# faasm/faabric

Hardware: NVIDIA H100
Metric: mpi_allreduce_resnet50_grads_algbw_GBps (higher is better)
Workload: dtype int32

## Files before the change

### csrc/kernels/coll_group.cuh

```cuda
#pragma once

#include "fb_prims.cuh"
#include "launch_api.h"

namespace fb {

__device__ __forceinline__ bool groupEnter(const GroupArgs& a,
                                           GroupSeg* sSegs,
                                           BlockBarrier& bar)
{
    const Vec16* src = reinterpret_cast<const Vec16*>(a.segs);
    Vec16* dst = reinterpret_cast<Vec16*>(sSegs);
    for (uint32_t i = threadIdx.x; i < a.nSegs * 2; i += blockDim.x) {
        dst[i] = src[i];
    }
    bar.epoch = 0;
    if (!a.noSync) {
        bar.load(a.comm);
        return bar.sync(a.comm);
    }
    __syncthreads();
    return true;
}

__device__ __forceinline__ void groupExit(const GroupArgs& a, BlockBarrier& bar)
{
    if (!a.noSync) {
        bar.sync(a.comm);
        bar.store(a.comm);
    }
}

__device__ __forceinline__ int groupSegOf(const GroupSeg* s,
                                          uint32_t nSegs,
                                          int cur,
                                          uint32_t ch)
{
    if (s[cur].chunk0 <= ch && (cur + 1 == (int)nSegs || ch < s[cur + 1].chunk0)) {
        return cur;
    }
    int lo = 0;
    int hi = (int)nSegs - 1;
    while (lo < hi) {
        int mid = (lo + hi + 1) >> 1;
        if (s[mid].chunk0 <= ch) {
            lo = mid;
        } else {
            hi = mid - 1;
        }
    }
    return lo;
}

}
```

### csrc/kernels/coll_move.cu

```cuda
#include "coll_group.cuh"
#include "coll_move.cuh"

namespace fb {

template<int W>
struct Word;
template<>
struct Word<16>
{
    using type = Vec16;
    __device__ __forceinline__ static Vec16 ld(const uint8_t* p)
    {
        return ldVecStream(p);
    }
    __device__ __forceinline__ static void st(uint8_t* p, const Vec16& v)
    {
        stVec(p, v);
    }
};
template<>
struct Word<4>
{
    using type = uint32_t;
    __device__ __forceinline__ static uint32_t ld(const uint8_t* p)
// ... 157 lines not shown
                    const uint8_t* src = (p == a.root)
                                           ? a.comm.heap[p] + a.sendOff + b
                                           : a.comm.heap[p] + a.recvOff + b;
                    gridCopy<W>(a.comm.heap[rank] + a.recvOff + b,
                                src,
                                e - b,
                                tid,
                                nthreads);
                }
            }
        }
    }
    if (!a.noSync) {
        bar.sync(a.comm);
    }
    bar.store(a.comm);
}

template<int W>
static cudaError_t launchMoveW(const MoveArgs& a,
                               int blocks,
                               int threads,
                               cudaStream_t s)
{
    int n = a.comm.nranks;
    if (n == 2) {
        moveKernel<W, 2><<<blocks, threads, 0, s>>>(a);
    } else if (n == 4) {
        moveKernel<W, 4><<<blocks, threads, 0, s>>>(a);
    } else if (n == 8) {
        moveKernel<W, 8><<<blocks, threads, 0, s>>>(a);
    } else {
        moveKernel<W, 0><<<blocks, threads, 0, s>>>(a);
    }
    return cudaGetLastError();
}

cudaError_t launchMove(const MoveArgs& a,
                       int width,
                       int blocks,
                       int threads,
                       cudaStream_t s)
{
    if (width == 16) {
        return launchMoveW<16>(a, blocks, threads, s);
    }
    if (width == 4) {
        return launchMoveW<4>(a, blocks, threads, s);
    }
    return launchMoveW<1>(a, blocks, threads, s);
}

template<int NR>
__global__ void __launch_bounds__(512, 1) groupAllGatherKernel(const GroupArgs a)
{
    extern __shared__ __align__(16) uint8_t sGroupRaw[];
    GroupSeg* sSegs = reinterpret_cast<GroupSeg*>(sGroupRaw);
    const FbCommDev& c = a.comm;
    const int n = (NR > 0) ? NR : c.nranks;
    BlockBarrier bar;
    const bool ok = groupEnter(a, sSegs, bar);

    if (ok && a.nSegs > 0) {
        constexpr int UNROLL = (NR == 8) ? 2 : (NR == 1 ? 8 : 4);
        constexpr uint32_t CHUNK = 32u * UNROLL;
        const uint32_t lane = threadIdx.x & 31;
        const uint32_t warpsPerCta = blockDim.x >> 5;
        const uint32_t warpStride = gridDim.x * warpsPerCta;
        const uint8_t* const in = c.heap[c.rank];
        int cur = 0;
        for (uint32_t ch = blockIdx.x * warpsPerCta + (threadIdx.x >> 5);
             ch < a.totalChunks;
             ch += warpStride) {
            cur = groupSegOf(sSegs, a.nSegs, cur, ch);
            const GroupSeg sg = sSegs[cur];
            const uint32_t v0 = (ch - sg.chunk0) * CHUNK;
            const uint8_t* const src = in + sg.sendOff + (uint64_t)v0 * 16;
            const uint64_t rOff = sg.recvOff + (uint64_t)v0 * 16;
            const uint32_t rem = sg.nVec - v0;
            if (rem >= CHUNK) {
                Vec16 v[UNROLL];
#pragma unroll
                for (int u = 0; u < UNROLL; u++) {
                    v[u] = ldVecStream(src + (uint64_t)(u * 32 + lane) * 16);
                }
                if constexpr (NR > 0) {
#pragma unroll
                    for (int p = 0; p < NR; p++) {
#pragma unroll
                        for (int u = 0; u < UNROLL; u++) {
                            stVec(c.heap[p] + rOff + (uint64_t)(u * 32 + lane) * 16, v[u]);
                        }
                    }
                } else {
                    for (int p = 0; p < n; p++) {
#pragma unroll
                        for (int u = 0; u < UNROLL; u++) {
                            stVec(c.heap[p] + rOff + (uint64_t)(u * 32 + lane) * 16, v[u]);
                        }
                    }
                }
            } else {
#pragma unroll
                for (int u = 0; u < UNROLL; u++) {
                    const uint32_t i = (uint32_t)u * 32 + lane;
                    if (i < rem) {
                        const Vec16 v = ldVecStream(src + (uint64_t)i * 16);
                        for (int p = 0; p < n; p++) {
                            stVec(c.heap[p] + rOff + (uint64_t)i * 16, v);
                        }
                    }
                }
            }
        }
    }
    groupExit(a, bar);
}

cudaError_t launchGroupAllGather(const GroupArgs& a,
                                 int blocks,
                                 int threads,
                                 cudaStream_t s)
{
    const size_t smem = (size_t)a.nSegs * sizeof(GroupSeg);
    const int n = a.comm.nranks;
    if (n == 1) {
        groupAllGatherKernel<1><<<blocks, threads, smem, s>>>(a);
    } else if (n == 2) {
        groupAllGatherKernel<2><<<blocks, threads, smem, s>>>(a);
    } else if (n == 4) {
        groupAllGatherKernel<4><<<blocks, threads, smem, s>>>(a);
    } else if (n == 8) {
        groupAllGatherKernel<8><<<blocks, threads, smem, s>>>(a);
    } else {
        groupAllGatherKernel<0><<<blocks, threads, smem, s>>>(a);
    }
    return cudaGetLastError();
}

__global__ void barrierKernel(const FbCommDev c)
{
    BlockBarrier bar;
    bar.load(c);
    bar.sync(c);
    bar.store(c);
}

cudaError_t launchBarrier(const FbCommDev& c, cudaStream_t s)
{
    barrierKernel<<<1, 32, 0, s>>>(c);
    return cudaGetLastError();
}

__device__ __forceinline__ bool lastBlockDone(uint32_t* counter)
{
    __shared__ int sLast;
    __syncthreads();
    if (threadIdx.x == 0) {
        __threadfence();
        uint32_t prev = atomicAdd(counter, 1u);
        sLast = (prev == gridDim.x - 1) ? 1 : 0;
        if (sLast) {
            *counter = 0;
            __threadfence();
        }
    }
    __syncthreads();
    return sLast != 0;
}

template<int W>
__global__ void __launch_bounds__(512, 1) p2pSendKernel(const P2PArgs a)
{
    const FbCommDev& c = a.comm;
    const uint64_t tid = (uint64_t)blockIdx.x * blockDim.x + threadIdx.x;
    const uint64_t nthreads = (uint64_t)gridDim.x * blockDim.x;
    if (a.stage) {
        uint8_t* dst = c.heap[c.rank] + a.srcOff;
        const uint64_t lenW = a.bytes - (a.bytes % W);
        gridCopy<W>(dst, a.local, lenW, tid, nthreads);
        if (tid == 0) {
            for (uint64_t b = lenW; b < a.bytes; b++) {
                dst[b] = a.local[b];
            }
        }
    }
    uint32_t* done = c.sig[c.rank] + FB_P2P_DONE_OFF + a.peer;
    if (lastBlockDone(done) && threadIdx.x == 0) {
        uint32_t* desc = reinterpret_cast<uint32_t*>(c.heap[a.peer] + a.descOff) +
                         ((uint32_t)c.rank * FB_P2P_RING + (a.seq % FB_P2P_RING)) * 4;
// ... 188 lines not shown
```

### csrc/kernels/coll_reduce.cuh

```cuda
#pragma once

#include "coll_group.cuh"
#include "fb_prims.cuh"
#include "launch_api.h"

namespace fb {

template<typename VR, int NR>
__device__ __forceinline__ Vec16 gatherReduce(const ReduceArgs& a,
                                              uint64_t byteOff)
{
    if constexpr (NR > 0) {
        Vec16 v[NR];
#pragma unroll
        for (int p = 0; p < NR; p++) {
            v[p] = ldVecStream(a.comm.heap[p] + a.sendOff + byteOff);
        }
        Vec16 acc = v[0];
#pragma unroll
        for (int p = 1; p < NR; p++) {
            acc = VR::apply(acc, v[p]);
        }
        return acc;
    } else {
// ... 315 lines not shown
    } else {
        Vec16 v = ldVec(p);
        memcpy(&out, &v, 16);
    }
    return out;
}

template<typename E>
__device__ __forceinline__ void stElemGlobal(uint8_t* p, const E& in)
{
    if constexpr (sizeof(E) == 1) {
        uint8_t v;
        memcpy(&v, &in, 1);
        *reinterpret_cast<volatile uint8_t*>(p) = v;
    } else if constexpr (sizeof(E) == 2) {
        uint16_t v;
        memcpy(&v, &in, 2);
        *reinterpret_cast<volatile uint16_t*>(p) = v;
    } else if constexpr (sizeof(E) == 4) {
        uint32_t v;
        memcpy(&v, &in, 4);
        *reinterpret_cast<volatile uint32_t*>(p) = v;
    } else if constexpr (sizeof(E) == 8) {
        uint64_t v;
        memcpy(&v, &in, 8);
        *reinterpret_cast<volatile uint64_t*>(p) = v;
    } else {
        Vec16 v;
        memcpy(&v, &in, 16);
        stVec(p, v);
    }
}

template<typename VR>
__device__ __forceinline__ void groupTail(const FbCommDev& c,
                                          const GroupSeg& sg,
                                          int n)
{
    using Elem = typename VR::Elem;
    constexpr uint32_t EB = VR::ELEM_BYTES;
    const uint64_t base = (uint64_t)sg.nVec * 16;
    for (uint32_t e = 0; e + EB <= sg.tailBytes; e += EB) {
        Elem acc = ldElemGlobal<Elem>(c.heap[0] + sg.sendOff + base + e);
        for (int p = 1; p < n; p++) {
            Elem v = ldElemGlobal<Elem>(c.heap[p] + sg.sendOff + base + e);
            acc = VR::combine(acc, v);
        }
        for (int p = 0; p < n; p++) {
            stElemGlobal<Elem>(c.heap[p] + sg.recvOff + base + e, acc);
        }
    }
}

template<typename VR, int NR>
__global__ void __launch_bounds__(512, 1) groupAllReduceKernel(
  const GroupArgs a)
{
    extern __shared__ __align__(16) uint8_t sGroupRaw[];
    GroupSeg* sSegs = reinterpret_cast<GroupSeg*>(sGroupRaw);
    const FbCommDev& c = a.comm;
    const int n = (NR > 0) ? NR : c.nranks;
    {
        const Vec16* src = reinterpret_cast<const Vec16*>(a.segs);
        Vec16* dst = reinterpret_cast<Vec16*>(sGroupRaw);
        for (uint32_t i = threadIdx.x; i < a.nSegs * 2; i += blockDim.x) {
            dst[i] = src[i];
        }
    }
    BlockBarrier bar;
    bar.epoch = 0;
    bool ok = true;
    if (!a.noSync) {
        bar.load(c);
        ok = bar.sync(c);
    } else {
        __syncthreads();
    }

    if (ok && a.nSegs > 0) {
        constexpr int UNROLL = (NR == 8) ? 2 : (NR == 1 ? 8 : 4);
        constexpr uint32_t CHUNK = 32u * UNROLL;
        const uint32_t lane = threadIdx.x & 31;
        const uint32_t warpsPerCta = blockDim.x >> 5;
        const uint32_t warpStride = gridDim.x * warpsPerCta;
        int cur = 0;
        for (uint32_t ch = blockIdx.x * warpsPerCta + (threadIdx.x >> 5);
             ch < a.totalChunks;
             ch += warpStride) {
            if (!(sSegs[cur].chunk0 <= ch &&
                  (cur + 1 == (int)a.nSegs || ch < sSegs[cur + 1].chunk0))) {
                int lo = 0;
                int hi = (int)a.nSegs - 1;
                while (lo < hi) {
                    int mid = (lo + hi + 1) >> 1;
                    if (sSegs[mid].chunk0 <= ch) {
                        lo = mid;
                    } else {
                        hi = mid - 1;
                    }
                }
                cur = lo;
            }
            const GroupSeg sg = sSegs[cur];
            const uint32_t v0 = (ch - sg.chunk0) * CHUNK;
            const uint64_t sOff = sg.sendOff + (uint64_t)v0 * 16;
            const uint64_t rOff = sg.recvOff + (uint64_t)v0 * 16;
            const uint32_t rem = sg.nVec > v0 ? sg.nVec - v0 : 0;
            if (rem >= CHUNK) {
                Vec16 acc[UNROLL];
                if constexpr (NR > 0) {
                    Vec16 v[UNROLL][NR];
#pragma unroll
                    for (int u = 0; u < UNROLL; u++) {
#pragma unroll
                        for (int p = 0; p < NR; p++) {
                            v[u][p] = ldVecStream(c.heap[p] + sOff +
                                                  (uint64_t)(u * 32 + lane) * 16);
                        }
                    }
#pragma unroll
                    for (int u = 0; u < UNROLL; u++) {
                        acc[u] = v[u][0];
#pragma unroll
                        for (int p = 1; p < NR; p++) {
                            acc[u] = VR::apply(acc[u], v[u][p]);
                        }
                    }
#pragma unroll
                    for (int u = 0; u < UNROLL; u++) {
#pragma unroll
                        for (int p = 0; p < NR; p++) {
                            stVec(c.heap[p] + rOff + (uint64_t)(u * 32 + lane) * 16,
                                  acc[u]);
                        }
                    }
                } else {
#pragma unroll
                    for (int u = 0; u < UNROLL; u++) {
                        acc[u] = ldVecStream(c.heap[0] + sOff +
                                             (uint64_t)(u * 32 + lane) * 16);
                    }
                    for (int p = 1; p < n; p++) {
                        Vec16 v[UNROLL];
#pragma unroll
                        for (int u = 0; u < UNROLL; u++) {
                            v[u] = ldVecStream(c.heap[p] + sOff +
                                               (uint64_t)(u * 32 + lane) * 16);
                        }
#pragma unroll
                        for (int u = 0; u < UNROLL; u++) {
                            acc[u] = VR::apply(acc[u], v[u]);
                        }
                    }
                    for (int p = 0; p < n; p++) {
#pragma unroll
                        for (int u = 0; u < UNROLL; u++) {
                            stVec(c.heap[p] + rOff + (uint64_t)(u * 32 + lane) * 16,
                                  acc[u]);
                        }
                    }
                }
            } else {
#pragma unroll
                for (int u = 0; u < UNROLL; u++) {
                    const uint32_t i = (uint32_t)u * 32 + lane;
                    if (i < rem) {
                        Vec16 acc = ldVecStream(c.heap[0] + sOff + (uint64_t)i * 16);
                        for (int p = 1; p < n; p++) {
                            Vec16 v = ldVecStream(c.heap[p] + sOff + (uint64_t)i * 16);
                            acc = VR::apply(acc, v);
                        }
                        for (int p = 0; p < n; p++) {
                            stVec(c.heap[p] + rOff + (uint64_t)i * 16, acc);
                        }
                    }
                }
                if (sg.tailBytes != 0 && lane == 0 && v0 + CHUNK > sg.nVec) {
                    groupTail<VR>(c, sg, n);
                }
            }
        }
    }

    if (!a.noSync) {
        bar.sync(c);
        bar.store(c);
    }
}

template<typename VR>
cudaError_t launchGroup(const GroupArgs& a,
                        int blocks,
                        int threads,
                        cudaStream_t stream)
{
    const size_t smem = (size_t)a.nSegs * sizeof(GroupSeg);
    const int nr = a.comm.nranks;
    if (nr == 1) {
        groupAllReduceKernel<VR, 1><<<blocks, threads, smem, stream>>>(a);
    } else if (nr == 2) {
        groupAllReduceKernel<VR, 2><<<blocks, threads, smem, stream>>>(a);
    } else if (nr == 4) {
        groupAllReduceKernel<VR, 4><<<blocks, threads, smem, stream>>>(a);
    } else if (nr == 8) {
        groupAllReduceKernel<VR, 8><<<blocks, threads, smem, stream>>>(a);
    } else {
        groupAllReduceKernel<VR, 0><<<blocks, threads, smem, stream>>>(a);
    }
    return cudaGetLastError();
}

template<typename VR, int NR>
__global__ void __launch_bounds__(512, 1) groupReduceScatterKernel(
  const GroupArgs a)
{
    extern __shared__ __align__(16) uint8_t sGroupRaw[];
    GroupSeg* sSegs = reinterpret_cast<GroupSeg*>(sGroupRaw);
    const FbCommDev& c = a.comm;
    const int n = (NR > 0) ? NR : c.nranks;
    BlockBarrier bar;
    const bool ok = groupEnter(a, sSegs, bar);

    if (ok && a.nSegs > 0) {
        constexpr int UNROLL = (NR == 8) ? 2 : (NR == 1 ? 8 : 4);
        constexpr uint32_t CHUNK = 32u * UNROLL;
        const uint32_t lane = threadIdx.x & 31;
        const uint32_t warpsPerCta = blockDim.x >> 5;
        const uint32_t warpStride = gridDim.x * warpsPerCta;
        uint8_t* const out = c.heap[c.rank];
        int cur = 0;
        for (uint32_t ch = blockIdx.x * warpsPerCta + (threadIdx.x >> 5);
             ch < a.totalChunks;
             ch += warpStride) {
            cur = groupSegOf(sSegs, a.nSegs, cur, ch);
            const GroupSeg sg = sSegs[cur];
            const uint32_t v0 = (ch - sg.chunk0) * CHUNK;
            const uint64_t sOff = sg.sendOff + (uint64_t)v0 * 16;
            uint8_t* const dst = out + sg.recvOff + (uint64_t)v0 * 16;
            const uint32_t rem = sg.nVec - v0;
            if (rem >= CHUNK) {
                Vec16 acc[UNROLL];
                if constexpr (NR > 0) {
                    Vec16 v[UNROLL][NR];
#pragma unroll
                    for (int u = 0; u < UNROLL; u++) {
#pragma unroll
                        for (int p = 0; p < NR; p++) {
                            v[u][p] = ldVecStream(c.heap[p] + sOff +
                                                  (uint64_t)(u * 32 + lane) * 16);
                        }
                    }
#pragma unroll
                    for (int u = 0; u < UNROLL; u++) {
                        acc[u] = v[u][0];
#pragma unroll
                        for (int p = 1; p < NR; p++) {
                            acc[u] = VR::apply(acc[u], v[u][p]);
                        }
                    }
                } else {
#pragma unroll
                    for (int u = 0; u < UNROLL; u++) {
                        acc[u] = ldVecStream(c.heap[0] + sOff +
                                             (uint64_t)(u * 32 + lane) * 16);
                    }
                    for (int p = 1; p < n; p++) {
                        Vec16 v[UNROLL];
#pragma unroll
                        for (int u = 0; u < UNROLL; u++) {
                            v[u] = ldVecStream(c.heap[p] + sOff +
                                               (uint64_t)(u * 32 + lane) * 16);
                        }
#pragma unroll
                        for (int u = 0; u < UNROLL; u++) {
                            acc[u] = VR::apply(acc[u], v[u]);
                        }
                    }
                }
#pragma unroll
                for (int u = 0; u < UNROLL; u++) {
                    stVec(dst + (uint64_t)(u * 32 + lane) * 16, acc[u]);
                }
            } else {
#pragma unroll
                for (int u = 0; u < UNROLL; u++) {
                    const uint32_t i = (uint32_t)u * 32 + lane;
                    if (i < rem) {
                        Vec16 acc = ldVecStream(c.heap[0] + sOff + (uint64_t)i * 16);
                        for (int p = 1; p < n; p++) {
                            Vec16 v = ldVecStream(c.heap[p] + sOff + (uint64_t)i * 16);
                            acc = VR::apply(acc, v);
                        }
                        stVec(dst + (uint64_t)i * 16, acc);
                    }
                }
            }
        }
    }
    groupExit(a, bar);
}

template<typename VR>
cudaError_t launchGroupReduceScatter(const GroupArgs& a,
                                     int blocks,
                                     int threads,
                                     cudaStream_t stream)
{
    const size_t smem = (size_t)a.nSegs * sizeof(GroupSeg);
    const int nr = a.comm.nranks;
    if (nr == 1) {
        groupReduceScatterKernel<VR, 1><<<blocks, threads, smem, stream>>>(a);
    } else if (nr == 2) {
        groupReduceScatterKernel<VR, 2><<<blocks, threads, smem, stream>>>(a);
    } else if (nr == 4) {
        groupReduceScatterKernel<VR, 4><<<blocks, threads, smem, stream>>>(a);
    } else if (nr == 8) {
        groupReduceScatterKernel<VR, 8><<<blocks, threads, smem, stream>>>(a);
    } else {
        groupReduceScatterKernel<VR, 0><<<blocks, threads, smem, stream>>>(a);
    }
    return cudaGetLastError();
}

template<typename VR>
cudaError_t preloadReduce()
{
    cudaFuncAttributes a;
    cudaError_t e = cudaSuccess;
#define FB_PRELOAD(k)                                                          \
    if (e == cudaSuccess) {                                                    \
        e = cudaFuncGetAttributes(&a, k);                                      \
    }
    FB_PRELOAD((reduceKernel<VR, 0>))
    FB_PRELOAD((reduceKernel<VR, 2>))
    FB_PRELOAD((reduceKernel<VR, 4>))
    FB_PRELOAD((reduceKernel<VR, 8>))
    FB_PRELOAD((llAllReduceKernel<VR, 0>))
    FB_PRELOAD((llAllReduceKernel<VR, 2>))
    FB_PRELOAD((llAllReduceKernel<VR, 4>))
    FB_PRELOAD((llAllReduceKernel<VR, 8>))
    FB_PRELOAD((groupAllReduceKernel<VR, 0>))
    FB_PRELOAD((groupAllReduceKernel<VR, 1>))
    FB_PRELOAD((groupAllReduceKernel<VR, 2>))
    FB_PRELOAD((groupAllReduceKernel<VR, 4>))
    FB_PRELOAD((groupAllReduceKernel<VR, 8>))
    FB_PRELOAD((groupReduceScatterKernel<VR, 0>))
    FB_PRELOAD((groupReduceScatterKernel<VR, 1>))
    FB_PRELOAD((groupReduceScatterKernel<VR, 2>))
    FB_PRELOAD((groupReduceScatterKernel<VR, 4>))
    FB_PRELOAD((groupReduceScatterKernel<VR, 8>))
#undef FB_PRELOAD
    return e;
}

template<typename VR>
const ReduceLaunchers* launchersFor()
{
    static const ReduceLaunchers l = { &launchReduce<VR>,
                                       &launchLL<VR>,
                                       &launchGroup<VR>,
                                       &launchGroupReduceScatter<VR>,
                                       &preloadReduce<VR> };
    return &l;
}

}
```

### csrc/kernels/fb_prims.cuh

```cuda
#pragma once

#include <cuda_bf16.h>
#include <cuda_fp16.h>
#include <stdint.h>

#include <type_traits>

#include "faabric/device/comm_abi.h"

namespace fb {

__device__ __forceinline__ void stReleaseSys(uint32_t* p, uint32_t v)
{
    asm volatile("st.release.sys.global.u32 [%0], %1;" ::"l"(p), "r"(v)
                 : "memory");
}

__device__ __forceinline__ void stRelaxedSys(uint32_t* p, uint32_t v)
{
    asm volatile("st.relaxed.sys.global.u32 [%0], %1;" ::"l"(p), "r"(v)
                 : "memory");
}

__device__ __forceinline__ uint32_t ldAcquireSys(const uint32_t* p)
// ... 74 lines not shown

    __device__ __forceinline__ bool sync(const FbCommDev& c)
    {
        epoch += 1;
        __syncthreads();
        bool ok = true;
        if (threadIdx.x < (unsigned)c.nranks) {
            int peer = threadIdx.x;
            const size_t slot = (size_t)(c.blockBase + blockIdx.x);
            uint32_t* remote = c.sig[peer] + slot * FB_MAX_RANKS + c.rank;
            stReleaseSys(remote, epoch);
            const uint32_t* mine =
              c.sig[c.rank] + slot * FB_MAX_RANKS + peer;
            ok = waitFlagGe(c, mine, epoch, FB_ERR_BARRIER_TIMEOUT);
        }
        return __syncthreads_and(ok ? 1 : 0) != 0;
    }
};

struct alignas(16) Vec16
{
    uint32_t w[4];
};

__device__ __forceinline__ Vec16 ldVec(const void* p)
{
    Vec16 v;
    asm volatile("ld.global.v4.u32 {%0,%1,%2,%3}, [%4];"
                 : "=r"(v.w[0]), "=r"(v.w[1]), "=r"(v.w[2]), "=r"(v.w[3])
                 : "l"(p)
                 : "memory");
    return v;
}

__device__ __forceinline__ Vec16 ldVecStream(const void* p)
{
    Vec16 v;
    asm volatile(
      "ld.global.L1::no_allocate.v4.u32 {%0,%1,%2,%3}, [%4];"
      : "=r"(v.w[0]), "=r"(v.w[1]), "=r"(v.w[2]), "=r"(v.w[3])
      : "l"(p)
      : "memory");
    return v;
}

__device__ __forceinline__ void stVec(void* p, const Vec16& v)
{
    asm volatile("st.global.v4.u32 [%0], {%1,%2,%3,%4};" ::"l"(p),
                 "r"(v.w[0]),
                 "r"(v.w[1]),
                 "r"(v.w[2]),
                 "r"(v.w[3])
                 : "memory");
}

template<int OP>
struct OpTag
{
    static constexpr int value = OP;
};

template<typename T>
struct PairVI
{
    T v;
    int32_t i;
};

template<typename T, int OP>
struct Reducer
{
    __device__ __forceinline__ static T apply(T a, T b)
    {
        if constexpr (OP == FB_OP_MAX && std::is_same_v<T, float>) {
            return fmaxf(a, b);
        } else if constexpr (OP == FB_OP_MAX && std::is_same_v<T, double>) {
            return fmax(a, b);
        } else if constexpr (OP == FB_OP_MIN && std::is_same_v<T, float>) {
            return fminf(a, b);
        } else if constexpr (OP == FB_OP_MIN && std::is_same_v<T, double>) {
            return fmin(a, b);
        } else if constexpr (OP == FB_OP_MAX) {
            return a > b ? a : b;
        } else if constexpr (OP == FB_OP_MIN) {
            return a < b ? a : b;
        } else if constexpr (OP == FB_OP_SUM) {
            return a + b;
        } else if constexpr (OP == FB_OP_PROD) {
            return a * b;
        } else if constexpr (OP == FB_OP_LAND) {
            return (T)((a != (T)0) && (b != (T)0));
        } else if constexpr (OP == FB_OP_LOR) {
            return (T)((a != (T)0) || (b != (T)0));
        } else if constexpr (OP == FB_OP_LXOR) {
            return (T)((a != (T)0) != (b != (T)0));
        } else {
            return a;
        }
    }
};

template<typename T, int OP>
__device__ __forceinline__ T bitOp(T a, T b)
{
    if constexpr (OP == FB_OP_BAND) {
        return a & b;
// ... 29 lines not shown
{
    static constexpr bool value = true;
};

template<int OP>
struct IsBitwiseOp
{
    static constexpr bool value =
      (OP == FB_OP_BAND || OP == FB_OP_BOR || OP == FB_OP_BXOR);
};

template<typename H, int OP>
__device__ __forceinline__ H halfLikeApply(H a, H b)
{
    float r = Reducer<float, OP>::apply((float)a, (float)b);
    return (H)r;
}

template<typename T, int OP>
__device__ __forceinline__ T reduceElem(T a, T b)
{
    if constexpr (IsBitwiseOp<OP>::value) {
        if constexpr (IsFloatLike<T>::value) {
            return a;
        } else {
            return bitOp<T, OP>(a, b);
        }
    } else if constexpr (sizeof(T) == 2 && IsFloatLike<T>::value) {
        return halfLikeApply<T, OP>(a, b);
    } else {
        return Reducer<T, OP>::apply(a, b);
    }
}

template<typename T, int OP>
__device__ __forceinline__ PairVI<T> reducePair(PairVI<T> a, PairVI<T> b)
{
    if constexpr (OP == FB_OP_MAXLOC) {
        if (b.v > a.v || (b.v == a.v && b.i < a.i)) {
            return b;
        }
        return a;
    } else {
        if (b.v < a.v || (b.v == a.v && b.i < a.i)) {
            return b;
        }
        return a;
    }
}

template<typename T, int OP>
__device__ __forceinline__ Vec16 reduceVec(const Vec16& a, const Vec16& b)
{
    constexpr int N = 16 / sizeof(T);
    union U
    {
        Vec16 v;
        T e[N];
        __device__ U() {}
    };
    U ua, ub, ur;
    ua.v = a;
    ub.v = b;
#pragma unroll
    for (int i = 0; i < N; i++) {
        ur.e[i] = reduceElem<T, OP>(ua.e[i], ub.e[i]);
    }
    return ur.v;
}

template<typename T, int OP>
__device__ __forceinline__ Vec16 reduceVecPair(const Vec16& a, const Vec16& b)
{
    using P = PairVI<T>;
    constexpr int N = 16 / sizeof(P);
    union U
    {
        Vec16 v;
        P e[N];
        __device__ U() {}
    };
    U ua, ub, ur;
    ua.v = a;
    ub.v = b;
#pragma unroll
    for (int i = 0; i < N; i++) {
        ur.e[i] = reducePair<T, OP>(ua.e[i], ub.e[i]);
    }
    return ur.v;
}

template<typename T, bool PAIR>
struct ElemOf
{
    using type = T;
};
template<typename T>
struct ElemOf<T, true>
{
    using type = PairVI<T>;
};

template<typename T, int OP, bool PAIR>
struct VecReduce
{
    static constexpr int ELEM_BYTES = PAIR ? sizeof(PairVI<T>) : sizeof(T);
// ... 42 lines not shown
```

### csrc/kernels/launch_api.h

```cpp
#pragma once

#include <cuda_runtime.h>
#include <stdint.h>

#include "faabric/device/comm_abi.h"

namespace fb {

#define FB_NUM_SMS 132

struct ReduceArgs
{
    FbCommDev comm;
    uint64_t sendOff;
    uint64_t recvOff;
    uint8_t* recvLocal;
    uint64_t bytes;
    uint64_t vecBegin;
    uint64_t vecEnd;
    uint64_t outBase;
    int32_t readRanks;
    uint32_t pushMask;
    int32_t tailOwner;
    int32_t noSync;
};

typedef cudaError_t (*ReduceLaunchFn)(const ReduceArgs& a,
                                      int nr,
                                      int blocks,
                                      int threads,
                                      cudaStream_t stream);

#define FB_LL_BLOCKS 8
#define FB_LL_THREADS 512
#define FB_LL_MAX_VECS (FB_LL_BLOCKS * FB_LL_THREADS)
#define FB_LL_MAX_BYTES (FB_LL_MAX_VECS * 16)
#define FB_LL_AREA_BYTES(nranks) ((uint64_t)2 * (nranks) * FB_LL_MAX_VECS * 32)

struct LLArgs
{
    FbCommDev comm;
    const uint8_t* sendLocal;
    uint8_t* recvLocal;
    uint64_t bytes;
    uint64_t llOff;
    int32_t byteAccess;
    int32_t pad;
};

typedef cudaError_t (*LLLaunchFn)(const LLArgs& a, cudaStream_t stream);

struct GroupSeg
{
    uint64_t sendOff;
    uint64_t recvOff;
    uint32_t nVec;
    uint32_t chunk0;
    uint32_t tailBytes;
    uint32_t pad;
};

struct GroupArgs
{
    FbCommDev comm;
    const GroupSeg* segs;
    uint32_t nSegs;
    uint32_t totalChunks;
    int32_t noSync;
    int32_t pad;
};

static inline int fbGroupUnroll(int nranks)
{
    return (nranks == 8) ? 2 : (nranks == 1 ? 8 : 4);
}
static inline uint32_t fbGroupChunkVecs(int nranks)
{
    return 32u * (uint32_t)fbGroupUnroll(nranks);
}
#define FB_GROUP_MAX_SEGS 1024

typedef cudaError_t (*GroupLaunchFn)(const GroupArgs& a,
                                     int blocks,
                                     int threads,
                                     cudaStream_t stream);

cudaError_t launchGroupAllGather(const GroupArgs& a,
                                 int blocks,
                                 int threads,
                                 cudaStream_t stream);

struct ReduceLaunchers
{
    ReduceLaunchFn reduce;
    LLLaunchFn ll;
    GroupLaunchFn group;
    GroupLaunchFn groupRs;
    cudaError_t (*preload)();
};

const ReduceLaunchers* findReduceLaunchers(int dtype, int op);
const ReduceLaunchers* findReduceLaunchersInt(int dtype, int op);
const ReduceLaunchers* findReduceLaunchersFloat(int dtype, int op);
const ReduceLaunchers* findReduceLaunchersPair(int dtype, int op);


enum MoveMode
{
    MOVE_ALLGATHER = 0,
    MOVE_ALLTOALL = 1,
    MOVE_GATHER = 2,
    MOVE_SCATTER = 3,
    MOVE_BCAST = 4,
    MOVE_BCAST_2STEP = 5
};

struct MoveArgs
{
    FbCommDev comm;
    uint64_t sendOff;
    uint64_t recvOff;
    uint8_t* recvLocal;
    uint64_t chunkBytes;
    uint64_t srcStride;
    uint64_t dstStride;
    int32_t mode;
    int32_t root;
// ... 234 lines not shown
```

### csrc/src/device/communicator.cpp

```cpp
#include "faabric/device/communicator.h"
#include "faabric/device/nvtx.h"

#include "faabric/device/bootstrap.h"
#include "faabric/device/cuda_driver.h"
#include "launch_api.h"
#include "loopback_kernels.h"

#include <algorithm>
#include <chrono>
#include <thread>
#include <cstdio>
#include <initializer_list>
#include <barrier>
#include <cstdlib>
#include <cstring>
#include <set>
#include <shared_mutex>
#include <stdexcept>
#include <unistd.h>

namespace faabric::device {

#define CUDA_OK(expr)                                                          \
    do {                                                                       \
// ... 1892 lines not shown
        rc = FB_E_UNSUPPORTED;
        return nullptr;
    }
    const size_t esize = fbDtypeSize(dtype);
    if (esize == 0 || kind < GROUP_ALLREDUCE || kind > GROUP_ALLGATHER) {
        rc = FB_E_INVALID;
        return nullptr;
    }
    bindDevice();
    auto plan = std::make_shared<GroupPlan>();
    plan->kind = kind;
    plan->dtype = dtype;
    plan->device = device_;
    plan->items = nItems;
    for (size_t begin = 0; begin < nItems; begin += GROUP_ITEMS_PER_LAUNCH) {
        const size_t cnt = std::min(GROUP_ITEMS_PER_LAUNCH, nItems - begin);
        SegBuild sb;
        rc = buildSegs(*this, kind, items + begin, cnt, esize, sb);
        if (rc != FB_OK) {
            return nullptr;
        }
        GroupLaunch l;
        l.nSegs = (uint32_t)sb.segs.size();
        l.totalChunks = sb.totalChunks;
        l.vecsPerRank = sb.vecsPerRank;
        l.bytes = sb.bytes;
        const size_t tb = std::max<size_t>(sb.segs.size(), 1) * sizeof(fb::GroupSeg);
        if (loop_) {
            plan->hostTables = true;
            l.dSegs = (fb::GroupSeg*)::malloc(tb);
            if (!sb.segs.empty()) {
                memcpy(l.dSegs, sb.segs.data(), sb.segs.size() * sizeof(fb::GroupSeg));
            }
            plan->launches.push_back(l);
            continue;
        }
        if (cudaMalloc((void**)&l.dSegs, tb) != cudaSuccess) {
            cudaGetLastError();
            rc = FB_E_CUDA;
            return nullptr;
        }
        plan->launches.push_back(l);
        if (!sb.segs.empty() &&
            cudaMemcpy(l.dSegs, sb.segs.data(), sb.segs.size() * sizeof(fb::GroupSeg), cudaMemcpyHostToDevice) !=
              cudaSuccess) {
            cudaGetLastError();
            rc = FB_E_CUDA;
            return nullptr;
        }
    }
    return plan;
}

static int groupGrid(const CommConfig& cfg, int nranks, uint64_t vecsPerRank)
{
    const int slots = nranks == 1 ? 2 * FB_NUM_SMS : FB_MAX_BLOCKS / cfg.channels;
    const int cap = std::min(slots, cfg.groupBlocks > 0 ? cfg.groupBlocks : (nranks == 1 ? 2 * FB_NUM_SMS : 128));
    const uint64_t warps = (uint64_t)cfg.threads / 32;
    const uint64_t chunks = (vecsPerRank + fb::fbGroupChunkVecs(nranks) - 1) / fb::fbGroupChunkVecs(nranks);
    const uint64_t want = (chunks + warps * 2 - 1) / (warps * 2);
    return (int)std::clamp<uint64_t>(want, 1, (uint64_t)cap);
}

int Communicator::launchGroup(const GroupLaunch& l, GroupKind kind, int dtype, int op, int flags, cudaStream_t s)
{
    const int n = dev_.nranks;
    const bool ss = streamSync_ && !(flags & FB_FLAG_NOSYNC) && n > 1;
    fb::GroupArgs a;
    memset(&a, 0, sizeof(a));
    a.comm = devFor(flags);
    a.segs = l.dSegs;
    a.nSegs = l.nSegs;
    a.totalChunks = l.totalChunks;
    a.noSync = ((flags & FB_FLAG_NOSYNC) || ss || n == 1) ? 1 : 0;
    if (ss && streamBarrier(flags, s) != FB_OK) {
        return FB_E_CUDA;
    }
    const int blocks = groupGrid(cfg_, n, l.vecsPerRank);
    cudaError_t e;
    if (kind == GROUP_REDUCE_SCATTER) {
        e = k_->groupReduceScatter(a, dtype, op, blocks, cfg_.threads, s);
    } else if (kind == GROUP_ALLGATHER) {
        e = k_->groupAllGather(a, blocks, cfg_.threads, s);
    } else {
        e = k_->group(a, dtype, op, blocks, cfg_.threads, s);
    }
    if (e != cudaSuccess) {
        return FB_E_CUDA;
    }
    if (ss && streamBarrier(flags, s) != FB_OK) {
        return FB_E_CUDA;
    }
    stats_.launches++;
    stats_.bytes += l.bytes;
    if (kind == GROUP_ALLREDUCE) {
        stats_.algoCount[FB_ALGO_TWOSHOT]++;
    }
    return FB_OK;
}

int Communicator::allReduceGroup(const GroupPlan& plan, int op, int flags, cudaStream_t s)
{
    NvtxRange nvtxRange("fb::allReduceGroup");
    if (parent_ != nullptr) {
        return FB_E_UNSUPPORTED;
    }
    if (plan.kind != GROUP_ALLREDUCE) {
        return FB_E_INVALID;
    }
    const fb::ReduceLaunchers* L = fb::findReduceLaunchers(plan.dtype, op);
    if (L == nullptr || L->group == nullptr) {
        return FB_E_UNSUPPORTED;
    }
    bindDevice();
    for (const auto& l : plan.launches) {
        int rc = launchGroup(l, GROUP_ALLREDUCE, plan.dtype, op, flags, s);
        if (rc != FB_OK) {
            return rc;
        }
    }
    lastAlgo_ = FB_ALGO_TWOSHOT;
    return FB_OK;
}

int Communicator::reduceScatterGroup(const GroupPlan& plan, int op, int flags, cudaStream_t s)
{
    NvtxRange nvtxRange("fb::reduceScatterGroup");
    if (parent_ != nullptr) {
        return FB_E_UNSUPPORTED;
    }
    if (plan.kind != GROUP_REDUCE_SCATTER) {
// ... 938 lines not shown
```

Measured before the change: 1342.

## Unify group kernels with software-pipelined walk, PDL launch, and larger grids

Measured after the change: 1384, median of 6. 3.2% higher.

```diff
diff --git a/csrc/kernels/coll_group.cuh b/csrc/kernels/coll_group.cuh
--- a/csrc/kernels/coll_group.cuh
+++ b/csrc/kernels/coll_group.cuh
@@ -9,6 +9,8 @@
                                            GroupSeg* sSegs,
                                            BlockBarrier& bar)
 {
+    asm volatile("griddepcontrol.launch_dependents;" ::: "memory");
+    asm volatile("griddepcontrol.wait;" ::: "memory");
     const Vec16* src = reinterpret_cast<const Vec16*>(a.segs);
     Vec16* dst = reinterpret_cast<Vec16*>(sSegs);
     for (uint32_t i = threadIdx.x; i < a.nSegs * 2; i += blockDim.x) {
@@ -52,4 +54,85 @@
     return lo;
 }
 
+template<typename Kernel>
+cudaError_t launchGroupKernel(Kernel kernel,
+                              const GroupArgs& a,
+                              int blocks,
+                              int threads,
+                              size_t smem,
+                              cudaStream_t stream)
+{
+    cudaLaunchConfig_t cfg = {};
+    cfg.gridDim = dim3((unsigned)blocks);
+    cfg.blockDim = dim3((unsigned)threads);
+    cfg.dynamicSmemBytes = smem;
+    cfg.stream = stream;
+    cudaLaunchAttribute attr[1];
+    attr[0].id = cudaLaunchAttributeProgrammaticStreamSerialization;
+    attr[0].val.programmaticStreamSerializationAllowed = 1;
+    cfg.attrs = attr;
+    cfg.numAttrs = 1;
+    return cudaLaunchKernelEx(&cfg, kernel, a);
 }
+
+__host__ __device__ constexpr bool groupPipelined(int nr)
+{
+    return nr == 1 || nr == 2;
+}
+
+template<int U, int NR>
+struct GroupStage
+{
+    Vec16 v[U][NR > 0 ? NR : 1];
+};
+
+template<int U, bool PIPE, typename Stage, typename Load, typename Store, typename Ragged>
+__device__ __forceinline__ void groupWalk(const GroupArgs& a,
+                                          const GroupSeg* sSegs,
+                                          Load load,
+                                          Store store,
+                                          Ragged ragged)
+{
+    constexpr uint32_t CHUNK = 32u * U;
+    const uint32_t warpsPerCta = blockDim.x >> 5;
+    const uint32_t warpStride = gridDim.x * warpsPerCta;
+    Stage held;
+    uint64_t heldOff = 0;
+    bool have = false;
+    int cur = 0;
+    for (uint32_t ch = blockIdx.x * warpsPerCta + (threadIdx.x >> 5);
+         ch < a.totalChunks;
+         ch += warpStride) {
+        cur = groupSegOf(sSegs, a.nSegs, cur, ch);
+        const GroupSeg sg = sSegs[cur];
+        const uint32_t v0 = (ch - sg.chunk0) * CHUNK;
+        const uint32_t rem = sg.nVec > v0 ? sg.nVec - v0 : 0;
+        if (rem < CHUNK) {
+            ragged(sg, v0, rem);
+            continue;
+        }
+        const uint64_t sOff = sg.sendOff + (uint64_t)v0 * 16;
+        const uint64_t rOff = sg.recvOff + (uint64_t)v0 * 16;
+        if constexpr (PIPE) {
+            Stage next;
+            load(next, sOff);
+            if (have) {
+                store(held, heldOff);
+            }
+            held = next;
+            heldOff = rOff;
+            have = true;
+        } else {
+            Stage s;
+            load(s, sOff);
+            store(s, rOff);
+        }
+    }
+    if constexpr (PIPE) {
+        if (have) {
+            store(held, heldOff);
+        }
+    }
+}
+
+}
diff --git a/csrc/kernels/coll_move.cu b/csrc/kernels/coll_move.cu
--- a/csrc/kernels/coll_move.cu
+++ b/csrc/kernels/coll_move.cu
@@ -233,7 +233,8 @@
 }
 
 template<int NR>
-__global__ void __launch_bounds__(512, 1) groupAllGatherKernel(const GroupArgs a)
+__global__ void __launch_bounds__(512, groupPipelined(NR) ? 2 : 1) groupAllGatherKernel(
+  const GroupArgs a)
 {
     extern __shared__ __align__(16) uint8_t sGroupRaw[];
     GroupSeg* sSegs = reinterpret_cast<GroupSeg*>(sGroupRaw);
@@ -243,57 +244,40 @@
     const bool ok = groupEnter(a, sSegs, bar);
 
     if (ok && a.nSegs > 0) {
-        constexpr int UNROLL = (NR == 8) ? 2 : (NR == 1 ? 8 : 4);
-        constexpr uint32_t CHUNK = 32u * UNROLL;
+        constexpr int U = fbGroupUnroll(NR);
+        using Stage = GroupStage<U, 1>;
         const uint32_t lane = threadIdx.x & 31;
-        const uint32_t warpsPerCta = blockDim.x >> 5;
-        const uint32_t warpStride = gridDim.x * warpsPerCta;
         const uint8_t* const in = c.heap[c.rank];
-        int cur = 0;
-        for (uint32_t ch = blockIdx.x * warpsPerCta + (threadIdx.x >> 5);
-             ch < a.totalChunks;
-             ch += warpStride) {
-            cur = groupSegOf(sSegs, a.nSegs, cur, ch);
-            const GroupSeg sg = sSegs[cur];
-            const uint32_t v0 = (ch - sg.chunk0) * CHUNK;
-            const uint8_t* const src = in + sg.sendOff + (uint64_t)v0 * 16;
-            const uint64_t rOff = sg.recvOff + (uint64_t)v0 * 16;
-            const uint32_t rem = sg.nVec - v0;
-            if (rem >= CHUNK) {
-                Vec16 v[UNROLL];
-#pragma unroll
-                for (int u = 0; u < UNROLL; u++) {
-                    v[u] = ldVecStream(src + (uint64_t)(u * 32 + lane) * 16);
-                }
-                if constexpr (NR > 0) {
-#pragma unroll
-                    for (int p = 0; p < NR; p++) {
-#pragma unroll
-                        for (int u = 0; u < UNROLL; u++) {
-                            stVec(c.heap[p] + rOff + (uint64_t)(u * 32 + lane) * 16, v[u]);
-                        }
-                    }
-                } else {
-                    for (int p = 0; p < n; p++) {
-#pragma unroll
-                        for (int u = 0; u < UNROLL; u++) {
-                            stVec(c.heap[p] + rOff + (uint64_t)(u * 32 + lane) * 16, v[u]);
-                        }
-                    }
-                }
-            } else {
-#pragma unroll
-                for (int u = 0; u < UNROLL; u++) {
-                    const uint32_t i = (uint32_t)u * 32 + lane;
-                    if (i < rem) {
-                        const Vec16 v = ldVecStream(src + (uint64_t)i * 16);
-                        for (int p = 0; p < n; p++) {
-                            stVec(c.heap[p] + rOff + (uint64_t)i * 16, v);
-                        }
-                    }
-                }
-            }
-        }
+        groupWalk<U, groupPipelined(NR), Stage>(
+          a,
+          sSegs,
+          [&](Stage& s, uint64_t sOff) {
+#pragma unroll
+              for (int u = 0; u < U; u++) {
+                  s.v[u][0] = ldVecData(in + sOff + (uint64_t)(u * 32 + lane) * 16);
+              }
+          },
+          [&](const Stage& s, uint64_t rOff) {
+              for (int p = 0; p < n; p++) {
+#pragma unroll
+                  for (int u = 0; u < U; u++) {
+                      stVecData(c.heap[p] + rOff + (uint64_t)(u * 32 + lane) * 16, s.v[u][0]);
+                  }
+              }
+          },
+          [&](const GroupSeg& sg, uint32_t v0, uint32_t rem) {
+#pragma unroll
+              for (int u = 0; u < U; u++) {
+                  const uint32_t i = (uint32_t)u * 32 + lane;
+                  if (i < rem) {
+                      const uint64_t vOff = (uint64_t)(v0 + i) * 16;
+                      const Vec16 v = ldVecData(in + sg.sendOff + vOff);
+                      for (int p = 0; p < n; p++) {
+                          stVecData(c.heap[p] + sg.recvOff + vOff, v);
+                      }
+                  }
+              }
+          });
     }
     groupExit(a, bar);
 }
@@ -306,17 +290,16 @@
     const size_t smem = (size_t)a.nSegs * sizeof(GroupSeg);
     const int n = a.comm.nranks;
     if (n == 1) {
-        groupAllGatherKernel<1><<<blocks, threads, smem, s>>>(a);
+        return launchGroupKernel(groupAllGatherKernel<1>, a, blocks, threads, smem, s);
     } else if (n == 2) {
-        groupAllGatherKernel<2><<<blocks, threads, smem, s>>>(a);
+        return launchGroupKernel(groupAllGatherKernel<2>, a, blocks, threads, smem, s);
     } else if (n == 4) {
-        groupAllGatherKernel<4><<<blocks, threads, smem, s>>>(a);
+        return launchGroupKernel(groupAllGatherKernel<4>, a, blocks, threads, smem, s);
     } else if (n == 8) {
-        groupAllGatherKernel<8><<<blocks, threads, smem, s>>>(a);
+        return launchGroupKernel(groupAllGatherKernel<8>, a, blocks, threads, smem, s);
     } else {
-        groupAllGatherKernel<0><<<blocks, threads, smem, s>>>(a);
-    }
-    return cudaGetLastError();
+        return launchGroupKernel(groupAllGatherKernel<0>, a, blocks, threads, smem, s);
+    }
 }
 
 __global__ void barrierKernel(const FbCommDev c)
diff --git a/csrc/kernels/coll_reduce.cuh b/csrc/kernels/coll_reduce.cuh
--- a/csrc/kernels/coll_reduce.cuh
+++ b/csrc/kernels/coll_reduce.cuh
@@ -391,166 +391,63 @@
     }
 }
 
+template<typename VR, int NR, int U>
+__device__ __forceinline__ void groupGather(GroupStage<U, NR>& s,
+                                            const FbCommDev& c,
+                                            int n,
+                                            uint64_t off)
+{
+    const uint32_t lane = threadIdx.x & 31;
+    if constexpr (NR > 0) {
+#pragma unroll
+        for (int u = 0; u < U; u++) {
+#pragma unroll
+            for (int p = 0; p < NR; p++) {
+                s.v[u][p] = ldVecData(c.heap[p] + off + (uint64_t)(u * 32 + lane) * 16);
+            }
+        }
+    } else {
+#pragma unroll
+        for (int u = 0; u < U; u++) {
+            s.v[u][0] = ldVecData(c.heap[0] + off + (uint64_t)(u * 32 + lane) * 16);
+        }
+        for (int p = 1; p < n; p++) {
+            Vec16 v[U];
+#pragma unroll
+            for (int u = 0; u < U; u++) {
+                v[u] = ldVecData(c.heap[p] + off + (uint64_t)(u * 32 + lane) * 16);
+            }
+#pragma unroll
+            for (int u = 0; u < U; u++) {
+                s.v[u][0] = VR::apply(s.v[u][0], v[u]);
+            }
+        }
+    }
+}
+
+template<typename VR, int NR, int U>
+__device__ __forceinline__ Vec16 groupReduced(const GroupStage<U, NR>& s, int u)
+{
+    Vec16 acc = s.v[u][0];
+#pragma unroll
+    for (int p = 1; p < NR; p++) {
+        acc = VR::apply(acc, s.v[u][p]);
+    }
+    return acc;
+}
+
+template<typename VR>
+__device__ __forceinline__ Vec16 groupGatherOne(const FbCommDev& c, int n, uint64_t off)
+{
+    Vec16 acc = ldVecData(c.heap[0] + off);
+    for (int p = 1; p < n; p++) {
+        acc = VR::apply(acc, ldVecData(c.heap[p] + off));
+    }
+    return acc;
+}
+
 template<typename VR, int NR>
-__global__ void __launch_bounds__(512, 1) groupAllReduceKernel(
-  const GroupArgs a)
-{
-    extern __shared__ __align__(16) uint8_t sGroupRaw[];
-    GroupSeg* sSegs = reinterpret_cast<GroupSeg*>(sGroupRaw);
-    const FbCommDev& c = a.comm;
-    const int n = (NR > 0) ? NR : c.nranks;
-    {
-        const Vec16* src = reinterpret_cast<const Vec16*>(a.segs);
-        Vec16* dst = reinterpret_cast<Vec16*>(sGroupRaw);
-        for (uint32_t i = threadIdx.x; i < a.nSegs * 2; i += blockDim.x) {
-            dst[i] = src[i];
-        }
-    }
-    BlockBarrier bar;
-    bar.epoch = 0;
-    bool ok = true;
-    if (!a.noSync) {
-        bar.load(c);
-        ok = bar.sync(c);
-    } else {
-        __syncthreads();
-    }
-
-    if (ok && a.nSegs > 0) {
-        constexpr int UNROLL = (NR == 8) ? 2 : (NR == 1 ? 8 : 4);
-        constexpr uint32_t CHUNK = 32u * UNROLL;
-        const uint32_t lane = threadIdx.x & 31;
-        const uint32_t warpsPerCta = blockDim.x >> 5;
-        const uint32_t warpStride = gridDim.x * warpsPerCta;
-        int cur = 0;
-        for (uint32_t ch = blockIdx.x * warpsPerCta + (threadIdx.x >> 5);
-             ch < a.totalChunks;
-             ch += warpStride) {
-            if (!(sSegs[cur].chunk0 <= ch &&
-                  (cur + 1 == (int)a.nSegs || ch < sSegs[cur + 1].chunk0))) {
-                int lo = 0;
-                int hi = (int)a.nSegs - 1;
-                while (lo < hi) {
-                    int mid = (lo + hi + 1) >> 1;
-                    if (sSegs[mid].chunk0 <= ch) {
-                        lo = mid;
-                    } else {
-                        hi = mid - 1;
-                    }
-                }
-                cur = lo;
-            }
-            const GroupSeg sg = sSegs[cur];
-            const uint32_t v0 = (ch - sg.chunk0) * CHUNK;
-            const uint64_t sOff = sg.sendOff + (uint64_t)v0 * 16;
-            const uint64_t rOff = sg.recvOff + (uint64_t)v0 * 16;
-            const uint32_t rem = sg.nVec > v0 ? sg.nVec - v0 : 0;
-            if (rem >= CHUNK) {
-                Vec16 acc[UNROLL];
-                if constexpr (NR > 0) {
-                    Vec16 v[UNROLL][NR];
-#pragma unroll
-                    for (int u = 0; u < UNROLL; u++) {
-#pragma unroll
-                        for (int p = 0; p < NR; p++) {
-                            v[u][p] = ldVecStream(c.heap[p] + sOff +
-                                                  (uint64_t)(u * 32 + lane) * 16);
-                        }
-                    }
-#pragma unroll
-                    for (int u = 0; u < UNROLL; u++) {
-                        acc[u] = v[u][0];
-#pragma unroll
-                        for (int p = 1; p < NR; p++) {
-                            acc[u] = VR::apply(acc[u], v[u][p]);
-                        }
-                    }
-#pragma unroll
-                    for (int u = 0; u < UNROLL; u++) {
-#pragma unroll
-                        for (int p = 0; p < NR; p++) {
-                            stVec(c.heap[p] + rOff + (uint64_t)(u * 32 + lane) * 16,
-                                  acc[u]);
-                        }
-                    }
-                } else {
-#pragma unroll
-                    for (int u = 0; u < UNROLL; u++) {
-                        acc[u] = ldVecStream(c.heap[0] + sOff +
-                                             (uint64_t)(u * 32 + lane) * 16);
-                    }
-                    for (int p = 1; p < n; p++) {
-                        Vec16 v[UNROLL];
-#pragma unroll
-                        for (int u = 0; u < UNROLL; u++) {
-                            v[u] = ldVecStream(c.heap[p] + sOff +
-                                               (uint64_t)(u * 32 + lane) * 16);
-                        }
-#pragma unroll
-                        for (int u = 0; u < UNROLL; u++) {
-                            acc[u] = VR::apply(acc[u], v[u]);
-                        }
-                    }
-                    for (int p = 0; p < n; p++) {
-#pragma unroll
-                        for (int u = 0; u < UNROLL; u++) {
-                            stVec(c.heap[p] + rOff + (uint64_t)(u * 32 + lane) * 16,
-                                  acc[u]);
-                        }
-                    }
-                }
-            } else {
-#pragma unroll
-                for (int u = 0; u < UNROLL; u++) {
-                    const uint32_t i = (uint32_t)u * 32 + lane;
-                    if (i < rem) {
-                        Vec16 acc = ldVecStream(c.heap[0] + sOff + (uint64_t)i * 16);
-                        for (int p = 1; p < n; p++) {
-                            Vec16 v = ldVecStream(c.heap[p] + sOff + (uint64_t)i * 16);
-                            acc = VR::apply(acc, v);
-                        }
-                        for (int p = 0; p < n; p++) {
-                            stVec(c.heap[p] + rOff + (uint64_t)i * 16, acc);
-                        }
-                    }
-                }
-                if (sg.tailBytes != 0 && lane == 0 && v0 + CHUNK > sg.nVec) {
-                    groupTail<VR>(c, sg, n);
-                }
-            }
-        }
-    }
-
-    if (!a.noSync) {
-        bar.sync(c);
-        bar.store(c);
-    }
-}
-
-template<typename VR>
-cudaError_t launchGroup(const GroupArgs& a,
-                        int blocks,
-                        int threads,
-                        cudaStream_t stream)
-{
-    const size_t smem = (size_t)a.nSegs * sizeof(GroupSeg);
-    const int nr = a.comm.nranks;
-    if (nr == 1) {
-        groupAllReduceKernel<VR, 1><<<blocks, threads, smem, stream>>>(a);
-    } else if (nr == 2) {
-        groupAllReduceKernel<VR, 2><<<blocks, threads, smem, stream>>>(a);
-    } else if (nr == 4) {
-        groupAllReduceKernel<VR, 4><<<blocks, threads, smem, stream>>>(a);
-    } else if (nr == 8) {
-        groupAllReduceKernel<VR, 8><<<blocks, threads, smem, stream>>>(a);
-    } else {
-        groupAllReduceKernel<VR, 0><<<blocks, threads, smem, stream>>>(a);
-    }
-    return cudaGetLastError();
-}
-
-template<typename VR, int NR>
-__global__ void __launch_bounds__(512, 1) groupReduceScatterKernel(
+__global__ void __launch_bounds__(512, groupPipelined(NR) ? 2 : 1) groupAllReduceKernel(
   const GroupArgs a)
 {
     extern __shared__ __align__(16) uint8_t sGroupRaw[];
@@ -561,80 +458,101 @@
     const bool ok = groupEnter(a, sSegs, bar);
 
     if (ok && a.nSegs > 0) {
-        constexpr int UNROLL = (NR == 8) ? 2 : (NR == 1 ? 8 : 4);
-        constexpr uint32_t CHUNK = 32u * UNROLL;
+        constexpr int U = fbGroupUnroll(NR);
+        using Stage = GroupStage<U, NR>;
         const uint32_t lane = threadIdx.x & 31;
-        const uint32_t warpsPerCta = blockDim.x >> 5;
-        const uint32_t warpStride = gridDim.x * warpsPerCta;
+        groupWalk<U, groupPipelined(NR), Stage>(
+          a,
+          sSegs,
+          [&](Stage& s, uint64_t sOff) { groupGather<VR, NR, U>(s, c, n, sOff); },
+          [&](const Stage& s, uint64_t rOff) {
+#pragma unroll
+              for (int u = 0; u < U; u++) {
+                  const Vec16 acc = groupReduced<VR, NR, U>(s, u);
+                  for (int p = 0; p < n; p++) {
+                      stVecData(c.heap[p] + rOff + (uint64_t)(u * 32 + lane) * 16, acc);
+                  }
+              }
+          },
+          [&](const GroupSeg& sg, uint32_t v0, uint32_t rem) {
+#pragma unroll
+              for (int u = 0; u < U; u++) {
+                  const uint32_t i = (uint32_t)u * 32 + lane;
+                  if (i < rem) {
+                      const uint64_t vOff = (uint64_t)(v0 + i) * 16;
+                      const Vec16 acc = groupGatherOne<VR>(c, n, sg.sendOff + vOff);
+                      for (int p = 0; p < n; p++) {
+                          stVecData(c.heap[p] + sg.recvOff + vOff, acc);
+                      }
+                  }
+              }
+              if (sg.tailBytes != 0 && lane == 0 && v0 + 32u * U > sg.nVec) {
+                  groupTail<VR>(c, sg, n);
+              }
+          });
+    }
+    groupExit(a, bar);
+}
+
+template<typename VR>
+cudaError_t launchGroup(const GroupArgs& a,
+                        int blocks,
+                        int threads,
+                        cudaStream_t stream)
+{
+    const size_t smem = (size_t)a.nSegs * sizeof(GroupSeg);
+    const int nr = a.comm.nranks;
+    if (nr == 1) {
+        return launchGroupKernel(groupAllReduceKernel<VR, 1>, a, blocks, threads, smem, stream);
+    } else if (nr == 2) {
+        return launchGroupKernel(groupAllReduceKernel<VR, 2>, a, blocks, threads, smem, stream);
+    } else if (nr == 4) {
+        return launchGroupKernel(groupAllReduceKernel<VR, 4>, a, blocks, threads, smem, stream);
+    } else if (nr == 8) {
+        return launchGroupKernel(groupAllReduceKernel<VR, 8>, a, blocks, threads, smem, stream);
+    } else {
+        return launchGroupKernel(groupAllReduceKernel<VR, 0>, a, blocks, threads, smem, stream);
+    }
+}
+
+template<typename VR, int NR>
+__global__ void __launch_bounds__(512, groupPipelined(NR) ? 2 : 1) groupReduceScatterKernel(
+  const GroupArgs a)
+{
+    extern __shared__ __align__(16) uint8_t sGroupRaw[];
+    GroupSeg* sSegs = reinterpret_cast<GroupSeg*>(sGroupRaw);
+    const FbCommDev& c = a.comm;
+    const int n = (NR > 0) ? NR : c.nranks;
+    BlockBarrier bar;
+    const bool ok = groupEnter(a, sSegs, bar);
+
+    if (ok && a.nSegs > 0) {
+        constexpr int U = fbGroupUnroll(NR);
+        using Stage = GroupStage<U, NR>;
+        const uint32_t lane = threadIdx.x & 31;
         uint8_t* const out = c.heap[c.rank];
-        int cur = 0;
-        for (uint32_t ch = blockIdx.x * warpsPerCta + (threadIdx.x >> 5);
-             ch < a.totalChunks;
-             ch += warpStride) {
-            cur = groupSegOf(sSegs, a.nSegs, cur, ch);
-            const GroupSeg sg = sSegs[cur];
-            const uint32_t v0 = (ch - sg.chunk0) * CHUNK;
-            const uint64_t sOff = sg.sendOff + (uint64_t)v0 * 16;
-            uint8_t* const dst = out + sg.recvOff + (uint64_t)v0 * 16;
-            const uint32_t rem = sg.nVec - v0;
-            if (rem >= CHUNK) {
-                Vec16 acc[UNROLL];
-                if constexpr (NR > 0) {
-                    Vec16 v[UNROLL][NR];
-#pragma unroll
-                    for (int u = 0; u < UNROLL; u++) {
-#pragma unroll
-                        for (int p = 0; p < NR; p++) {
-                            v[u][p] = ldVecStream(c.heap[p] + sOff +
-                                                  (uint64_t)(u * 32 + lane) * 16);
-                        }
-                    }
-#pragma unroll
-                    for (int u = 0; u < UNROLL; u++) {
-                        acc[u] = v[u][0];
-#pragma unroll
-                        for (int p = 1; p < NR; p++) {
-                            acc[u] = VR::apply(acc[u], v[u][p]);
-                        }
-                    }
-                } else {
-#pragma unroll
-                    for (int u = 0; u < UNROLL; u++) {
-                        acc[u] = ldVecStream(c.heap[0] + sOff +
-                                             (uint64_t)(u * 32 + lane) * 16);
-                    }
-                    for (int p = 1; p < n; p++) {
-                        Vec16 v[UNROLL];
-#pragma unroll
-                        for (int u = 0; u < UNROLL; u++) {
-                            v[u] = ldVecStream(c.heap[p] + sOff +
-                                               (uint64_t)(u * 32 + lane) * 16);
-                        }
-#pragma unroll
-                        for (int u = 0; u < UNROLL; u++) {
-                            acc[u] = VR::apply(acc[u], v[u]);
-                        }
-                    }
-                }
-#pragma unroll
-                for (int u = 0; u < UNROLL; u++) {
-                    stVec(dst + (uint64_t)(u * 32 + lane) * 16, acc[u]);
-                }
-            } else {
-#pragma unroll
-                for (int u = 0; u < UNROLL; u++) {
-                    const uint32_t i = (uint32_t)u * 32 + lane;
-                    if (i < rem) {
-                        Vec16 acc = ldVecStream(c.heap[0] + sOff + (uint64_t)i * 16);
-                        for (int p = 1; p < n; p++) {
-                            Vec16 v = ldVecStream(c.heap[p] + sOff + (uint64_t)i * 16);
-                            acc = VR::apply(acc, v);
-                        }
-                        stVec(dst + (uint64_t)i * 16, acc);
-                    }
-                }
-            }
-        }
+        groupWalk<U, groupPipelined(NR), Stage>(
+          a,
+          sSegs,
+          [&](Stage& s, uint64_t sOff) { groupGather<VR, NR, U>(s, c, n, sOff); },
+          [&](const Stage& s, uint64_t rOff) {
+#pragma unroll
+              for (int u = 0; u < U; u++) {
+                  stVecData(out + rOff + (uint64_t)(u * 32 + lane) * 16,
+                             groupReduced<VR, NR, U>(s, u));
+              }
+          },
+          [&](const GroupSeg& sg, uint32_t v0, uint32_t rem) {
+#pragma unroll
+              for (int u = 0; u < U; u++) {
+                  const uint32_t i = (uint32_t)u * 32 + lane;
+                  if (i < rem) {
+                      const uint64_t vOff = (uint64_t)(v0 + i) * 16;
+                      stVecData(out + sg.recvOff + vOff,
+                                 groupGatherOne<VR>(c, n, sg.sendOff + vOff));
+                  }
+              }
+          });
     }
     groupExit(a, bar);
 }
@@ -648,17 +566,16 @@
     const size_t smem = (size_t)a.nSegs * sizeof(GroupSeg);
     const int nr = a.comm.nranks;
     if (nr == 1) {
-        groupReduceScatterKernel<VR, 1><<<blocks, threads, smem, stream>>>(a);
+        return launchGroupKernel(groupReduceScatterKernel<VR, 1>, a, blocks, threads, smem, stream);
     } else if (nr == 2) {
-        groupReduceScatterKernel<VR, 2><<<blocks, threads, smem, stream>>>(a);
+        return launchGroupKernel(groupReduceScatterKernel<VR, 2>, a, blocks, threads, smem, stream);
     } else if (nr == 4) {
-        groupReduceScatterKernel<VR, 4><<<blocks, threads, smem, stream>>>(a);
+        return launchGroupKernel(groupReduceScatterKernel<VR, 4>, a, blocks, threads, smem, stream);
     } else if (nr == 8) {
-        groupReduceScatterKernel<VR, 8><<<blocks, threads, smem, stream>>>(a);
-    } else {
-        groupReduceScatterKernel<VR, 0><<<blocks, threads, smem, stream>>>(a);
-    }
-    return cudaGetLastError();
+        return launchGroupKernel(groupReduceScatterKernel<VR, 8>, a, blocks, threads, smem, stream);
+    } else {
+        return launchGroupKernel(groupReduceScatterKernel<VR, 0>, a, blocks, threads, smem, stream);
+    }
 }
 
 template<typename VR>
diff --git a/csrc/kernels/fb_prims.cuh b/csrc/kernels/fb_prims.cuh
--- a/csrc/kernels/fb_prims.cuh
+++ b/csrc/kernels/fb_prims.cuh
@@ -150,6 +150,21 @@
                  "r"(v.w[2]),
                  "r"(v.w[3])
                  : "memory");
+}
+
+__device__ __forceinline__ Vec16 ldVecData(const uint8_t* p)
+{
+    Vec16 v;
+    asm("ld.global.L1::no_allocate.v4.u32 {%0,%1,%2,%3}, [%4];"
+        : "=r"(v.w[0]), "=r"(v.w[1]), "=r"(v.w[2]), "=r"(v.w[3])
+        : "l"(p));
+    return v;
+}
+
+__device__ __forceinline__ void stVecData(uint8_t* p, const Vec16& v)
+{
+    __builtin_assume(__isGlobal(p));
+    *reinterpret_cast<Vec16*>(p) = v;
 }
 
 template<int OP>
@@ -285,6 +300,19 @@
 template<typename T, int OP>
 __device__ __forceinline__ Vec16 reduceVec(const Vec16& a, const Vec16& b)
 {
+    if constexpr (sizeof(T) == 2 && !IsFloatLike<T>::value &&
+                  (OP == FB_OP_MAX || OP == FB_OP_MIN)) {
+        Vec16 r;
+#pragma unroll
+        for (int i = 0; i < 4; i++) {
+            if constexpr (std::is_signed_v<T>) {
+                r.w[i] = OP == FB_OP_MAX ? __vmaxs2(a.w[i], b.w[i]) : __vmins2(a.w[i], b.w[i]);
+            } else {
+                r.w[i] = OP == FB_OP_MAX ? __vmaxu2(a.w[i], b.w[i]) : __vminu2(a.w[i], b.w[i]);
+            }
+        }
+        return r;
+    }
     constexpr int N = 16 / sizeof(T);
     union U
     {
diff --git a/csrc/kernels/launch_api.h b/csrc/kernels/launch_api.h
--- a/csrc/kernels/launch_api.h
+++ b/csrc/kernels/launch_api.h
@@ -70,9 +70,9 @@
     int32_t pad;
 };
 
-static inline int fbGroupUnroll(int nranks)
-{
-    return (nranks == 8) ? 2 : (nranks == 1 ? 8 : 4);
+static constexpr int fbGroupUnroll(int nranks)
+{
+    return (nranks == 2 || nranks == 8) ? 2 : 4;
 }
 static inline uint32_t fbGroupChunkVecs(int nranks)
 {
diff --git a/csrc/src/device/communicator.cpp b/csrc/src/device/communicator.cpp
--- a/csrc/src/device/communicator.cpp
+++ b/csrc/src/device/communicator.cpp
@@ -1968,10 +1968,10 @@
     return plan;
 }
 
-static int groupGrid(const CommConfig& cfg, int nranks, uint64_t vecsPerRank)
-{
-    const int slots = nranks == 1 ? 2 * FB_NUM_SMS : FB_MAX_BLOCKS / cfg.channels;
-    const int cap = std::min(slots, cfg.groupBlocks > 0 ? cfg.groupBlocks : (nranks == 1 ? 2 * FB_NUM_SMS : 128));
+static int groupGrid(const CommConfig& cfg, int nranks, uint64_t vecsPerRank, bool noSync)
+{
+    const int slots = noSync ? 4 * FB_NUM_SMS : FB_MAX_BLOCKS / cfg.channels;
+    const int cap = std::min(slots, cfg.groupBlocks > 0 ? cfg.groupBlocks : (noSync ? 4 * FB_NUM_SMS : 128));
     const uint64_t warps = (uint64_t)cfg.threads / 32;
     const uint64_t chunks = (vecsPerRank + fb::fbGroupChunkVecs(nranks) - 1) / fb::fbGroupChunkVecs(nranks);
     const uint64_t want = (chunks + warps * 2 - 1) / (warps * 2);
@@ -1992,7 +1992,7 @@
     if (ss && streamBarrier(flags, s) != FB_OK) {
         return FB_E_CUDA;
     }
-    const int blocks = groupGrid(cfg_, n, l.vecsPerRank);
+    const int blocks = groupGrid(cfg_, n, l.vecsPerRank, a.noSync != 0);
     cudaError_t e;
     if (kind == GROUP_REDUCE_SCATTER) {
         e = k_->groupReduceScatter(a, dtype, op, blocks, cfg_.threads, s);
```
